# chrg127/stereomatching

Measured on AMD Instinct MI355X. Metric: Mpixel-disparities/s, higher is better.
Workload: dtype u32 bit-packed edges, i32 counts

## Files before the change

### stereomatching_amd/csrc/sm_bs_network.h

```cpp
#pragma once

#ifdef SM_BS_NETWORK_HOST
#include <cstdint>
typedef uint32_t u32;
#define SM_NET_FN inline
#define SM_NET_UNROLL
#define SM_PIN() do { } while (0)
#define SM_SYNC() do { } while (0)
template <int IMM>
inline u32 bop(u32 a, u32 b, u32 c)
{
    u32 r = 0;
    for (int k = 0; k < 8; k++)
        if ((IMM >> k) & 1) r |= ((k & 4) ? a : ~a) & ((k & 2) ? b : ~b) & ((k & 1) ? c : ~c);
    return r;
}
#else
#define SM_NET_FN __device__ __forceinline__
#define SM_NET_UNROLL _Pragma("unroll")
#endif

#include "sm_bs_ops.h"

struct NetCell { short a, b, c, s, cy; short imm; short w; bool grp = false; };

template <int N, int SB>
struct NetPlan {
    static constexpr int NIN = 2 * N + SB;
    static constexpr int MAXC = 2 * N + 2 * SB;
    NetCell cell[MAXC] = {};
    int ncell = 0;
    int nwires = NIN;
    int nops = 0;
    short out[SB] = {};
};

template <int N, int SB, bool GR = false>
constexpr NetPlan<N, SB> net_make_plan()
{
    NetPlan<N, SB> p;
    constexpr int G = GR ? N / 3 : 0;
    short q[4 * N + 4 * SB] = {}, nx[2 * N + 2 * SB] = {};
    bool qneg[4 * N + 4 * SB] = {}, nxneg[2 * N + 2 * SB] = {};
    short qgrp[4 * N + 4 * SB] = {};
    int head = 0, tail = 0, nn = 0;
    for (int w = 0; w < SB; w++) {
        const bool top = w == SB - 1;
        head = 0; tail = 0;
        q[tail] = (short)(2 * N + w); qneg[tail++] = false;
        if (w == 0) {
            for (int g = 0; g < G; g++) {
                qgrp[tail] = (short)(1 + 3 * g); qneg[tail++] = false;
                qgrp[tail] = (short)(1 + N + 3 * g); qneg[tail++] = true;
            }
            for (int i = 3 * G; i < N; i++) {
                q[tail] = (short)i; qneg[tail++] = false;
                q[tail] = (short)(N + i); qneg[tail++] = true;
            }
        }
        for (int i = 0; i < nn; i++) { q[tail] = nx[i]; qneg[tail++] = nxneg[i]; }
        nn = 0;
        while (tail - head >= 2) {
            const int k = tail - head >= 3 ? 3 : 2;
            for (int j = 0; j < k; j++)
                if (qgrp[head + j]) {
                    const short in0 = (short)(qgrp[head + j] - 1);
                    NetCell gc = {in0, (short)(in0 + 1), (short)(in0 + 2), -1, -1, BOP_MAJ_NC, (short)w, true};
                    gc.s = (short)p.nwires++;
                    gc.cy = (short)p.nwires++;
                    nx[nn] = gc.cy; nxneg[nn++] = qneg[head + j];
                    p.nops++;
                    q[head + j] = gc.s; qgrp[head + j] = 0;
                    p.cell[p.ncell++] = gc;
                }
            short in[3] = {-1, -1, -1};
            int np = 0, ng = 0;
            for (int j = 0; j < k; j++) if (!qneg[head + j]) in[np++] = q[head + j];
            for (int j = 0; j < k; j++) if (qneg[head + j]) in[np + ng++] = q[head + j];
            head += k;
            NetCell c = {in[0], in[1], in[2], (short)p.nwires++, -1, 0, (short)w};
            bool sneg = false, cneg = false;
            if (k == 3) {
                sneg = ng & 1; cneg = ng >= 2;
                c.imm = ng == 1 ? BOP_MAJ_NC : ng == 2 ? BOP_BORROW : BOP_MAJ;
            } else {
                sneg = ng == 2; cneg = ng >= 1;
                c.imm = ng == 1 ? BOP_ANDN : 0;
            }
            p.nops++;
            if (!top) {
                c.cy = (short)p.nwires++;
                nx[nn] = c.cy; nxneg[nn++] = cneg;
                p.nops++;
            }
            q[--head] = c.s; qneg[head] = sneg;
            p.cell[p.ncell++] = c;
        }
        p.out[w] = q[head];
        if (qneg[head] && !top) { nx[nn] = q[head]; nxneg[nn++] = true; }
    }
    bool made[NetPlan<N, SB>::NIN + 2 * NetPlan<N, SB>::MAXC] = {};
    for (int i = 0; i < NetPlan<N, SB>::NIN; i++) made[i] = true;
    NetCell order[NetPlan<N, SB>::MAXC] = {};
    bool done[NetPlan<N, SB>::MAXC] = {};
    for (int n = 0; n < p.ncell; n++) {
        int pick = -1;
        for (int i = 0; i < p.ncell; i++) {
            const NetCell &c = p.cell[i];
            if (done[i] || !made[c.a] || !made[c.b] || (c.c >= 0 && !made[c.c])) continue;
            if (pick < 0 || c.w > p.cell[pick].w) pick = i;
        }
        done[pick] = true;
        order[n] = p.cell[pick];
        made[order[n].s] = true;
        if (order[n].cy >= 0) made[order[n].cy] = true;
    }
    for (int n = 0; n < p.ncell; n++) p.cell[n] = order[n];
    return p;
}

template <int N, int SB, bool GR = false>
struct NetPlanOf { static constexpr NetPlan<N, SB> value = net_make_plan<N, SB, GR>(); };

template <int N, int SB, bool GR = false>
constexpr int net_min_distance(int it)
{
    const NetPlan<N, SB> p = NetPlanOf<N, SB, GR>::value;
    int pos[NetPlan<N, SB>::NIN + 2 * NetPlan<N, SB>::MAXC] = {};
    for (int i = 0; i < NetPlan<N, SB>::NIN; i++) pos[i] = -(1 << 20);
    int at = 0, best = 1 << 20;
    for (int n = 0; n < p.ncell; n++) {
        const NetCell &c = p.cell[n];
        const short in[3] = {c.a, c.b, c.c};
        for (int j = 0; j < 3; j++)
            if (in[j] >= 0 && at - pos[in[j]] < best) best = at - pos[in[j]];
        pos[c.s] = at;
        if (!c.grp) at += it;
        if (c.cy >= 0) { pos[c.cy] = at; at += it; }
    }
    return best;
}

template <int N, bool GR = false>
constexpr int net_ops() { return net_make_plan<N, bits_for(N * N), GR>().nops; }
constexpr int net_ops_count_tree(int n)
{
    int ops = 0, m = n;
    for (int w = 0; w < bits_for(n); w++) {
        int carries = 0;
        while (m >= 3) { ops += 2; m -= 2; carries++; }
        if (m == 2) { ops += 2; m = 1; carries++; }
        m = carries;
    }
    return ops;
}
constexpr int net_ops_addsub(int n)
{
    const int hb = bits_for(n), sb = bits_for(n * n);
    int ops = 2 + 2 * (hb - 1) + 2;
    for (int k = 1; k < sb; k++) ops += k + 1 < sb ? 2 : 1;
    return ops;
}
constexpr int net_ops_separate(int n) { return 2 * net_ops_count_tree(n) + net_ops_addsub(n); }

template <int N, int SB, int IT, int DS, int NW, int ID, typename XF>
SM_NET_FN u32 net_wire(const u32 (&S)[DS][SB], int dd0, XF &xin, const u32 (&wr)[IT][NW], int it)
{
    if constexpr (ID < 2 * N) return xin(it, ID);
    else if constexpr (ID < 2 * N + SB) return S[dd0 + it][ID - 2 * N];
    else return wr[it][ID - 2 * N - SB];
}

template <int N, int SB, int IT, int DS, bool GR, int C, int NW, typename XF>
SM_NET_FN void net_cells(u32 (&S)[DS][SB], int dd0, XF &xin, u32 (&wr)[IT][NW])
{
    constexpr NetPlan<N, SB> P = NetPlanOf<N, SB, GR>::value;
    if constexpr (C < P.ncell) {
        constexpr NetCell cl = P.cell[C];
        constexpr int NIN = 2 * N + SB;
        constexpr bool full = cl.c >= 0;
        u32 a[IT], b[IT], c[IT];
SM_NET_UNROLL
        for (int it = 0; it < IT; it++) {
            a[it] = net_wire<N, SB, IT, DS, NW, cl.a>(S, dd0, xin, wr, it);
            b[it] = net_wire<N, SB, IT, DS, NW, cl.b>(S, dd0, xin, wr, it);
            if constexpr (full) c[it] = net_wire<N, SB, IT, DS, NW, cl.c>(S, dd0, xin, wr, it);
            else c[it] = 0u;
        }
SM_NET_UNROLL
        for (int it = 0; it < IT; it++) {
            if constexpr (cl.grp) wr[it][cl.s - NIN] = c[it];
            else {
                if constexpr (full) wr[it][cl.s - NIN] = bop<BOP_XOR3>(a[it], b[it], c[it]);
                else wr[it][cl.s - NIN] = a[it] ^ b[it];
                SM_PIN();
            }
        }
        if constexpr (cl.cy >= 0) {
SM_NET_UNROLL
            for (int it = 0; it < IT; it++) {
                if constexpr (full || cl.imm != 0) wr[it][cl.cy - NIN] = bop<cl.imm>(a[it], b[it], c[it]);
                else wr[it][cl.cy - NIN] = a[it] & b[it];
                SM_PIN();
            }
        }
        SM_SYNC();
        net_cells<N, SB, IT, DS, GR, C + 1, NW>(S, dd0, xin, wr);
    }
}

template <int N, int SB, bool GR = false>
constexpr bool net_planes_from_cells()
{
    constexpr NetPlan<N, SB> P = NetPlanOf<N, SB, GR>::value;
    for (int k = 0; k < SB; k++)
        if (P.out[k] < 2 * N + SB) return false;
    return true;
}

template <int N, int SB, int IT, int DS, bool GR = false, typename XF>
SM_NET_FN void network_lockstep(u32 (&S)[DS][SB], int dd0, XF xin)
{
    constexpr NetPlan<N, SB> P = NetPlanOf<N, SB, GR>::value;
    constexpr int NIN = 2 * N + SB, NW = P.nwires - NIN;
    static_assert(net_planes_from_cells<N, SB, GR>(), "every plane of S' comes out of a cell");
    static_assert(net_min_distance<N, SB, GR>(IT) >= IT, "a cell reads a result made fewer than IT operations before");
    u32 wr[IT][NW];
    net_cells<N, SB, IT, DS, GR, 0, NW>(S, dd0, xin, wr);
SM_NET_UNROLL
    for (int k = 0; k < SB; k++)
SM_NET_UNROLL
        for (int it = 0; it < IT; it++) S[dd0 + it][k] = wr[it][P.out[k] - NIN];
}
```

### stereomatching_amd/csrc/sm_match_bs_kernel.h

```cpp

#pragma once
#include "sm_internal.h"

#ifndef SM_BS_TU
#error "define SM_BS_TU (a token naming the translation unit) before including this header"
#endif
#define SM_BS_CAT2(a, b) a##b
#define SM_BS_CAT(a, b) SM_BS_CAT2(a, b)

#define SM_BS_WAVES 2
#define SM_STAGE_CH_L 4
#define SM_STAGE_CH_R 5

#ifdef SM_STAMPS
static __device__ unsigned long long *g_sm_stamps;
int SM_BS_CAT(sm_bs_set_stamps_, SM_BS_TU)(void *buf)
{
    return hipMemcpyToSymbol(HIP_SYMBOL(g_sm_stamps), &buf, sizeof buf) == hipSuccess ? 0 : SM_ERR_HIP;
}
#define SM_STAMP(slot)                                                                          \
    do {                                                                                        \
        if ((threadIdx.x & 63) == 0 && g_sm_stamps) {                   \
            const size_t wg_ = (((size_t)blockIdx.z * gridDim.y + blockIdx.y) * gridDim.x + blockIdx.x) \
                               * (blockDim.x >> 6) + (threadIdx.x >> 6);                        \
            g_sm_stamps[wg_ * 10 + 2 * (slot)] = __builtin_amdgcn_s_memrealtime();              \
            g_sm_stamps[wg_ * 10 + 2 * (slot) + 1] = __builtin_amdgcn_s_memtime();              \
            if ((slot) == 0)                                                                    \
                g_sm_stamps[wg_ * 10 + 8] = ((unsigned long long)__builtin_amdgcn_s_getreg(63508) << 32) | \
                                            (unsigned)__builtin_amdgcn_s_getreg(63492);         \
        }                                                                                       \
    } while (0)
#else
#define SM_STAMP(slot) do { } while (0)
#endif

template <int IMM>
__device__ __forceinline__ u32 bop(u32 a, u32 b, u32 c)
{
    return __builtin_amdgcn_bitop3_b32(a, b, c, IMM);
}
#include "sm_bs_ops.h"

__device__ __forceinline__ u32 alignbit(u32 hi, u32 lo, u32 sh)
{
    return __builtin_amdgcn_alignbit(hi, lo, sh);
}

typedef unsigned long long u64;
struct RawRow { u64 l01; u32 l2; u64 r01, r23; };
struct RawCentre { u32 l; u64 r01; u32 r2; };
typedef __attribute__((address_space(3))) const volatile u32 lds_vu32;
typedef u64 __attribute__((aligned(4))) u64a4;
typedef __attribute__((address_space(3))) const volatile u64a4 lds_vu64;
__device__ __forceinline__ void lds_issue(RawRow &o, u32 aL, u32 aR)
{
    o.l01 = *(lds_vu64 *)(uintptr_t)aL;
    o.l2 = *(lds_vu32 *)(uintptr_t)(aL + 8);
    o.r01 = *(lds_vu64 *)(uintptr_t)aR;
    o.r23 = *(lds_vu64 *)(uintptr_t)(aR + 8);
}
__device__ __forceinline__ void lds_issue(RawCentre &o, u32 aL, u32 aR)
{
    o.l = *(lds_vu32 *)(uintptr_t)aL;
    o.r01 = *(lds_vu64 *)(uintptr_t)aR;
    o.r2 = *(lds_vu32 *)(uintptr_t)(aR + 8);
}

typedef int v4i __attribute__((ext_vector_type(4)));
__device__ __forceinline__ void store_map4(i32 *p, v4i v)
{
    asm volatile("global_store_dwordx4 %0, %1, off sc1\n\ts_nop 1" : : "v"(p), "v"(v) : "memory");
}

template <int SB, int HB>
__device__ __forceinline__ void add_planes(u32 (&s)[SB], const u32 (&h)[HB])
{
    u32 c = s[0] & h[0];
    s[0] ^= h[0];
#pragma unroll
    for (int k = 1; k < SB; k++) {
        if (k < HB) {
            const u32 cn = bop<BOP_MAJ>(s[k], h[k], c);
            s[k] = bop<BOP_XOR3>(s[k], h[k], c);
            c = cn;
        } else {
            const u32 cn = k + 1 < SB ? s[k] & c : 0u;
            s[k] ^= c;
            c = cn;
        }
    }
}

#define SM_PIN() __builtin_amdgcn_sched_barrier(0)
#define SM_SYNC() do { asm volatile("s_nop 0"); SM_PIN(); } while (0)

#include "sm_bs_network.h"

template <int N, int HB, int IT, typename XF>
__device__ __forceinline__ void count_lockstep(XF xin, u32 (&h)[IT][HB])
{
    u32 q[IT][2 * N + 2];
    int head = 0, tail = N;
#pragma unroll
    for (int w = 0; w < HB; w++) {
        u32 nx[IT][N + 1];
        int nn = 0;
#pragma unroll
        for (int adder = 0; adder < N; adder++) {
            if (tail - head >= 3) {
                u32 a[IT], b[IT], c[IT];
#pragma unroll
                for (int it = 0; it < IT; it++) {
                    const bool in0 = w == 0 && head < N, in1 = w == 0 && head + 1 < N, in2 = w == 0 && head + 2 < N;
                    a[it] = in0 ? xin(it, in0 ? head : 0) : q[it][head];
                    b[it] = in1 ? xin(it, in1 ? head + 1 : 0) : q[it][head + 1];
                    c[it] = in2 ? xin(it, in2 ? head + 2 : 0) : q[it][head + 2];
                }
#pragma unroll
                for (int it = 0; it < IT; it++) { q[it][tail] = bop<BOP_XOR3>(a[it], b[it], c[it]); SM_PIN(); }
#pragma unroll
                for (int it = 0; it < IT; it++) { nx[it][nn] = bop<BOP_MAJ>(a[it], b[it], c[it]); SM_PIN(); }
                SM_SYNC();
                head += 3; tail++; nn++;
            }
        }
        if (tail - head == 2) {
            u32 a[IT], b[IT];
#pragma unroll
            for (int it = 0; it < IT; it++) {
                const bool in0 = w == 0 && head < N, in1 = w == 0 && head + 1 < N;
                a[it] = in0 ? xin(it, in0 ? head : 0) : q[it][head];
                b[it] = in1 ? xin(it, in1 ? head + 1 : 0) : q[it][head + 1];
            }
#pragma unroll
            for (int it = 0; it < IT; it++) { q[it][tail] = a[it] ^ b[it]; SM_PIN(); }
#pragma unroll
            for (int it = 0; it < IT; it++) { nx[it][nn] = a[it] & b[it]; SM_PIN(); }
            head += 2; tail++; nn++;
        }
#pragma unroll
        for (int it = 0; it < IT; it++) {
            const bool in0 = w == 0 && head < N;
            h[it][w] = tail - head == 1 ? (in0 ? xin(it, in0 ? head : 0) : q[it][head]) : 0u;
        }
        head = 0; tail = 0;
#pragma unroll
        for (int i = 0; i < N + 1; i++)
            if (i < nn) {
#pragma unroll
                for (int it = 0; it < IT; it++) q[it][tail] = nx[it][i];
                tail++;
            }
    }
}

template <int SB, int HB, int GS, int DS>
__device__ __forceinline__ void add_lockstep(u32 (&S)[DS][SB], int dd0, const u32 (&h)[GS][HB])
{
    u32 c[GS];
#pragma unroll
    for (int g = 0; g < GS; g++) { c[g] = S[dd0 + g][0] & h[g][0]; SM_PIN(); }
#pragma unroll
    for (int g = 0; g < GS; g++) { S[dd0 + g][0] ^= h[g][0]; SM_PIN(); }
#pragma unroll
    for (int k = 1; k < SB; k++) {
        u32 cn[GS];
#pragma unroll
        for (int g = 0; g < GS; g++) {
            if (k + 1 < SB) { cn[g] = k < HB ? bop<BOP_MAJ>(S[dd0 + g][k], h[g][k], c[g]) : (S[dd0 + g][k] & c[g]); SM_PIN(); }
            else cn[g] = 0;
        }
#pragma unroll
        for (int g = 0; g < GS; g++) {
            if (k < HB) S[dd0 + g][k] = bop<BOP_XOR3>(S[dd0 + g][k], h[g][k], c[g]);
            else S[dd0 + g][k] ^= c[g];
            SM_PIN();
        }
#pragma unroll
        for (int g = 0; g < GS; g++) c[g] = cn[g];
        SM_SYNC();
    }
}

template <int V> struct IntTag { static constexpr int value = V; };

template <int T, int CH>
struct RowStager {
    const u32 *src;
    u32 *dst;
    int rw, total, step_k, step_from, wrap_from;
    int e, k, from;
    u32 v[CH];
    __device__ __forceinline__ RowStager(const u32 *src_, int stride, u32 *dst_, int nrow, int rw_)
        : src(src_), dst(dst_), rw(rw_), total(nrow * rw_)
    {
        const float inv = __builtin_amdgcn_rcpf((float)rw);
        const int t_row = (int)(((float)T + 0.5f) * inv), row = (int)(((float)threadIdx.x + 0.5f) * inv);
        step_k = T - t_row * rw;
        step_from = t_row * stride + step_k;
        wrap_from = stride - rw;
        e = (int)threadIdx.x;
        k = e - row * rw;
        from = row * stride + k;
    }
    __device__ __forceinline__ bool more() const { return e - (int)threadIdx.x + T * CH < total; }
    template <typename Tag>
    __device__ __forceinline__ void issue(Tag)
    {
#pragma unroll
        for (int j = 0; j < CH; j++) {
            v[j] = src[Tag::value && e >= total ? 0 : from];
            e += T; k += step_k; from += step_from;
            if (k >= rw) { k -= rw; from += wrap_from; }
        }
    }
    template <typename Tag>
    __device__ __forceinline__ void write(Tag) const
    {
#pragma unroll
        for (int j = 0; j < CH; j++) {
            const int ej = e - (CH - j) * T;
            dst[Tag::value && ej >= total ? 0 : ej] = v[j];
        }
    }
};

template <int CTRL>
__device__ __forceinline__ u32 dpp(u32 v)
{
    return (u32)__builtin_amdgcn_update_dpp(0, (int)v, CTRL, 0xf, 0xf, true);
}

template <int K>
__device__ __forceinline__ u32 from_partner(u32 v)
{
    if (K == 0) return dpp<0xB1>(v);
    if (K == 1) return dpp<0x4E>(v);
    if (K == 2) return dpp<0x141>(v);
    if (K == 3) return dpp<0x140>(v);
    return (u32)__shfl_xor((int)v, 1 << K);
}


template <int N, int DS, bool FULLD, bool GHOST, bool CAP2 = false, bool DUO = false>
__global__ __launch_bounds__(DUO ? 128 : 64, SM_BS_WAVES) void k_match_bs(const u32 *__restrict__ ext,
                                                 i32 *__restrict__ web, i32 *__restrict__ best,
                                                 const MatchGeom g)
{
    constexpr int HALF = N / 2;
    constexpr int HB = bits_for(N);
    constexpr int SB = bits_for(N * N);
    constexpr int AB = DS == 16 ? 4 : DS == 8 ? 3 : 2;
    constexpr int ABMAX = AB + 6;
    static_assert(SB <= 16, "window counts are moved through two byte lanes");
    static_assert((1 << SB) - 1 > N * N, "the all-ones marker must not be a real count");
    static_assert(N + DS - 1 + 31 < 96, "right window must fit three words");

    extern __shared__ __attribute__((aligned(16))) u32 lds[];
    if (CAP2) asm volatile("" ::: "v175");
    if (web == nullptr) return;
    const int tid = DUO ? (int)(threadIdx.x & 63u) : (int)threadIdx.x;
    const int wv = DUO ? __builtin_amdgcn_readfirstlane((int)(threadIdx.x >> 6)) : 0;
    const int pair = blockIdx.z;
    SM_STAMP(0);
    const unsigned slot_parity = __builtin_amdgcn_s_getreg(63492) & 1;
    unsigned long long clk = __builtin_amdgcn_s_memtime();
    constexpr unsigned PATTERN = DS == 16 ? 0xF0F0F0F0u : 0xAAAAAAAAu;
    const unsigned long long clk0 = clk;
#define SM_SLICE_PRIO()                                                               \
    do {                                                                              \
        const unsigned unit_ = (unsigned)((clk - clk0) >> 14) & 31u;                  \
        if (((PATTERN >> unit_) ^ slot_parity) & 1) __builtin_amdgcn_s_setprio(3);    \
        else __builtin_amdgcn_s_setprio(0);                                           \
    } while (0)
#define SM_SLICE_READ() do { clk = __builtin_amdgcn_s_memtime(); } while (0)
    int tile_x, tile_y;
    sm_xcd_tile(g.tiles_x, g.tiles_y, tile_x, tile_y);
    const int tx0 = tile_x * g.tw;
    const int ty0 = tile_y * (DUO ? 2 * g.tile_h : g.tile_h);
    const int plw = g.plw, prw = g.prw, nsr = g.nsr;
    const u32 *extL = ext + (size_t)pair * 2 * g.ext_image_words;
    u32 *pL = lds;
    u32 *pR = pL + nsr * plw;

    constexpr int T = DUO ? 128 : 64;
    const u32 *rowsL = extL + (size_t)ty0 * g.ext_words + (tx0 >> 5);
    RowStager<T, SM_STAGE_CH_L> stL(rowsL, g.ext_words, pL, nsr, plw);
    RowStager<T, SM_STAGE_CH_R> stR(rowsL + g.ext_image_words, g.ext_words, pR, nsr, prw);
    while (stL.more()) { stL.issue(IntTag<0>{}); stL.write(IntTag<0>{}); }
    stL.issue(IntTag<1>{});
    while (stR.more()) { stR.issue(IntTag<0>{}); stR.write(IntTag<0>{}); }
    stR.issue(IntTag<1>{});

    const int s = tid & (g.nl - 1);
    const int wi = tid >> g.log2nl;
    const int d0 = s * DS;
    const int x0 = tx0 + 32 * wi;
    const int bL = SM_PADT + 32 * wi - HALF, bR = bL + d0;
    const int wL = bL >> 5, shL = bL & 31, wR = bR >> 5, shR = bR & 31;
    const int bRc = SM_PADT + 32 * wi + d0;
    const int wRc = bRc >> 5, shRc = bRc & 31;
    const int wLc = 1 + wi;

    u32 cvv[N];
    if (GHOST) {
        const int lo = min(64, max(0, HALF - x0)), hi = min(64, max(0, g.w + HALF - x0));
        const unsigned long long below_hi = hi >= 64 ? ~0ull : (1ull << hi) - 1ull;
        const unsigned long long below_lo = lo >= 64 ? ~0ull : (1ull << lo) - 1ull;
        const unsigned long long cm = hi > lo ? below_hi & ~below_lo : 0ull;
        const u32 c0 = (u32)cm, c1 = (u32)(cm >> 32);
#pragma unroll
        for (int i = 0; i < N; i++) cvv[i] = i ? alignbit(c1, c0, i) : c0;
    }
    u32 dvalid = (1u << DS) - 1u;
    if (!FULLD) {
        const int dlim = g.D - d0;
        dvalid = dlim >= DS ? (1u << DS) - 1u : (dlim <= 0 ? 0u : ((1u << dlim) - 1u));
    }

    u32 S[DS][SB];
#pragma unroll
    for (int dd = 0; dd < DS; dd++)
#pragma unroll
        for (int k = 0; k < SB; k++) {
            S[dd][k] = 0;
            asm volatile("" : "+v"(S[dd][k]));
        }

    SM_PIN();
    stL.write(IntTag<1>{});
    stR.write(IntTag<1>{});
    __syncthreads();
    SM_STAMP(1);

    struct RowViews { u32 lv[N]; u32 rw[3]; };
    auto load_views = [&](int srow, RowViews &v) {
        const u32 *rl = pL + srow * plw + wL;
        const u32 *rr = pR + srow * prw + wR;
        const u32 l0 = alignbit(rl[1], rl[0], shL), l1 = alignbit(rl[2], rl[1], shL);
#pragma unroll
        for (int k = 0; k < 3; k++) v.rw[k] = alignbit(rr[k + 1], rr[k], shR);
#pragma unroll
        for (int i = 0; i < N; i++) v.lv[i] = i ? alignbit(l1, l0, i) : l0;
    };
    auto views_of = [&](const RawRow &q, RowViews &v) {
        const u32 a0 = (u32)q.l01, a1 = (u32)(q.l01 >> 32), a2 = q.l2;
        const u32 r0 = (u32)q.r01, r1 = (u32)(q.r01 >> 32), r2 = (u32)q.r23, r3 = (u32)(q.r23 >> 32);
        const u32 l0 = alignbit(a1, a0, shL), l1 = alignbit(a2, a1, shL);
        v.rw[0] = alignbit(r1, r0, shR); v.rw[1] = alignbit(r2, r1, shR); v.rw[2] = alignbit(r3, r2, shR);
#pragma unroll
        for (int i = 0; i < N; i++) v.lv[i] = i ? alignbit(l1, l0, i) : l0;
    };
    auto rview = [&](const RowViews &v, int j) -> u32 {
        return (j & 31) ? alignbit(v.rw[(j >> 5) + 1], v.rw[j >> 5], j & 31) : v.rw[j >> 5];
    };

    constexpr int GW = DS >= 4 ? 4 : DS;
    constexpr int GS = DS >= 4 ? 4 : DS;
    static_assert(DS % GW == 0 && DS % GS == 0, "shift groups");
    auto slide_in = [&](int srow) {
        RowViews v;
        load_views(srow, v);
        u32 rv[N + GW - 1];
#pragma unroll
        for (int m = 0; m < N - 1; m++) rv[m + GW] = rview(v, m);
#pragma unroll
        for (int dd0 = 0; dd0 < DS; dd0 += GW) {
#pragma unroll
            for (int m = 0; m < N - 1; m++) rv[m] = rv[m + GW];
#pragma unroll
            for (int m = 0; m < GW; m++) { rv[N - 1 + m] = rview(v, dd0 + N - 1 + m); SM_PIN(); }
            SM_SYNC();
            u32 h[GW][HB];
            count_lockstep<N, HB, GW>([&](int it, int i) -> u32 {
                const u32 x = GHOST ? bop<BOP_XOR_AND>(v.lv[i], rv[it + i], cvv[i]) : (v.lv[i] ^ rv[it + i]);
                SM_PIN();
                return x;
            }, h);
            add_lockstep<SB, HB, GW, DS>(S, dd0, h);
        }
    };
    constexpr int G = N / 3, RXK = 3 * (G - 1), RXW = RXK + GS;
    constexpr bool GROUPED = !GHOST && 2 * G * DS > 2 * G + 2 * (RXK + DS) && !(DS == 8 && N >= 19);
    auto slide_views = [&](const RowViews &vn, const RowViews &vo) {
        u32 rn[N + GS - 1], ro[N + GS - 1];
        u32 lxn[G], lxo[G], rxn[RXW], rxo[RXW];
#pragma unroll
        for (int m = 0; m < N - 1; m++) { rn[m + GS] = rview(vn, m); ro[m + GS] = rview(vo, m); }
        if (GROUPED) {
            SM_PIN(); SM_SYNC();
#pragma unroll
            for (int gq = 0; gq < G; gq++) {
                lxn[gq] = bop<BOP_XOR3>(vn.lv[3 * gq], vn.lv[3 * gq + 1], vn.lv[3 * gq + 2]); SM_PIN();
                lxo[gq] = bop<BOP_XOR3>(vo.lv[3 * gq], vo.lv[3 * gq + 1], vo.lv[3 * gq + 2]); SM_PIN();
            }
#pragma unroll
            for (int m = 0; m < RXK; m++) {
                rxn[m + GS] = bop<BOP_XOR3>(rn[m + GS], rn[m + GS + 1], rn[m + GS + 2]); SM_PIN();
                rxo[m + GS] = bop<BOP_XOR3>(ro[m + GS], ro[m + GS + 1], ro[m + GS + 2]); SM_PIN();
            }
        }
#pragma unroll
        for (int dd0 = 0; dd0 < DS; dd0 += GS) {
#pragma unroll
            for (int m = 0; m < N - 1; m++) { rn[m] = rn[m + GS]; ro[m] = ro[m + GS]; }
#pragma unroll
            for (int m = 0; m < GS; m++) {
                rn[N - 1 + m] = rview(vn, dd0 + N - 1 + m); SM_PIN();
                ro[N - 1 + m] = rview(vo, dd0 + N - 1 + m); SM_PIN();
            }
            SM_SYNC();
            if (GROUPED) {
#pragma unroll
                for (int m = 0; m < RXK; m++) { rxn[m] = rxn[m + GS]; rxo[m] = rxo[m + GS]; }
#pragma unroll
                for (int m = 0; m < GS; m++) { rxn[RXK + m] = bop<BOP_XOR3>(rn[RXK + m], rn[RXK + m + 1], rn[RXK + m + 2]); SM_PIN(); }
#pragma unroll
                for (int m = 0; m < GS; m++) { rxo[RXK + m] = bop<BOP_XOR3>(ro[RXK + m], ro[RXK + m + 1], ro[RXK + m + 2]); SM_PIN(); }
            }
            network_lockstep<N, SB, GS, DS, GROUPED>(S, dd0, [&](int it, int i) -> u32 {
                const int col = i < N ? i : i - N;
                if (GROUPED && col < 3 * G && col % 3 == 2) {
                    const u32 p = (i < N ? lxn[col / 3] : lxo[col / 3]) ^ (i < N ? rxn[it + col - 2] : rxo[it + col - 2]);
                    SM_PIN();
                    return p;
                }
                const u32 l = i < N ? vn.lv[col] : vo.lv[col];
                const u32 r = i < N ? rn[it + col] : ro[it + col];
                const u32 x = GHOST ? bop<BOP_XOR_AND>(l, r, cvv[col]) : (l ^ r);
                SM_PIN();
                return x;
            });
            SM_SYNC();
        }
    };

    const int mid = DUO ? min(ty0 + g.tile_h, g.h) : 0;
    const int sgn = DUO ? (wv ? 1 : -1) : 1;
    const int y0 = DUO ? (wv ? mid : mid - 1) : ty0;
    const int c0 = DUO ? y0 - ty0 + HALF : HALF;
    const int rows_out = DUO ? (wv ? min(ty0 + 2 * g.tile_h, g.h) - mid : mid - ty0)
                             : min(g.tile_h, g.h - ty0);

    SM_SLICE_PRIO();
    if (DUO) {
#pragma unroll 1
        for (int e = 0; e <= HALF; e++) {
        if (e == HALF) {
        constexpr int DH = DS / 2, XP = DH * SB / 2;
        static_assert(DS % 2 == 0 && (DH * SB) % 2 == 0, "exchange halves");
        typedef u32 v2u __attribute__((ext_vector_type(2)));
        v2u *xq = reinterpret_cast<v2u *>(lds + g.xm_off - XP * 128) + tid;
        auto exchange = [&](auto own_tag) {
            constexpr int OWN = decltype(own_tag)::value, OTH = 1 - OWN;
            v2u *slot_own = xq + OWN * XP * 64, *slot_oth = xq + OTH * XP * 64;
#pragma unroll
            for (int j = 0; j < XP; j++) {
                const int p = 2 * j, q = 2 * j + 1;
                const v2u v = {S[OTH * DH + p / SB][p % SB], S[OTH * DH + q / SB][q % SB]};
                slot_oth[j * 64] = v;
            }
            __syncthreads();
#pragma unroll
            for (int dd = 0; dd < DH; dd += 2) {
                u32 o[2][SB];
#pragma unroll
                for (int j = 0; j < SB; j++) {
                    const int p = 2 * j, q = 2 * j + 1;
                    const v2u v = slot_own[(dd * SB / 2 + j) * 64];
                    o[p / SB][p % SB] = v.x;
                    o[q / SB][q % SB] = v.y;
                }
                add_planes<SB, SB>(S[OWN * DH + dd], o[0]);
                add_planes<SB, SB>(S[OWN * DH + dd + 1], o[1]);
#pragma unroll
                for (int j = 0; j < SB; j++) {
                    const int p = 2 * j, q = 2 * j + 1;
                    const v2u v = {S[OWN * DH + dd + p / SB][p % SB], S[OWN * DH + dd + q / SB][q % SB]};
                    slot_own[(dd * SB / 2 + j) * 64] = v;
                }
            }
            __syncthreads();
#pragma unroll
            for (int j = 0; j < XP; j++) {
                const int p = 2 * j, q = 2 * j + 1;
                const v2u v = slot_oth[j * 64];
                S[OTH * DH + p / SB][p % SB] = v.x;
                S[OTH * DH + q / SB][q % SB] = v.y;
            }
        };
        if (wv) exchange(IntTag<1>{}); else exchange(IntTag<0>{});
        }
        slide_in(c0 + sgn * e);
        }
        if (rows_out <= 0) return;
    } else {
#pragma unroll 1
        for (int e = 0; e < N; e++) slide_in(e);
    }
    SM_SLICE_READ();
    SM_STAMP(2);

    u32 *xm_base = lds + g.xm_off - ((DUO && wv) ? g.xm_words : 0);
    u32 *xm_wbase = xm_base + (s & 3) * ((SB + AB + 3) / 4) * 256;
    const u32 xm_wunit = (u32)(wi * (g.nl >> 2) + (s >> 2) + 2 * (s & 3));
    const u32 ldsL = (u32)(uintptr_t)pL, ldsR = (u32)(uintptr_t)pR;
    const u32 sL = (u32)(sgn * 4 * plw), sR = (u32)(sgn * 4 * prw);
    u32 aNewL = ldsL + 4u * wL + sL * (HALF + 1) + 4u * plw * c0, aNewR = ldsR + 4u * wR + sR * (HALF + 1) + 4u * prw * c0;
    u32 aCenL = ldsL + 4u * wLc + 4u * plw * c0, aCenR = ldsR + 4u * wRc + 4u * prw * c0;
    RawRow qn, qo;
    RawCentre qc;
    lds_issue(qc, aCenL, aCenR);
    if (!DUO || rows_out > 1) {
        lds_issue(qn, aNewL, aNewR);
        lds_issue(qo, aNewL - sL * N, aNewR - sR * N);
    }
#pragma unroll 1
    for (int t = 0;;) {
        SM_SLICE_PRIO();
        const int y = y0 + sgn * t;
        const u32 lc = qc.l;
        const u32 c0_ = (u32)qc.r01, c1_ = (u32)(qc.r01 >> 32), c2_ = qc.r2;
        const u32 rc0 = alignbit(c1_, c0_, shRc), rc1 = alignbit(c2_, c1_, shRc);

        u32 B[SB], arg[ABMAX];
#pragma unroll
        for (int k = 0; k < ABMAX; k++) arg[k] = 0;
        {
            constexpr int Q = 4, QS = DS / Q;
            constexpr int AQ = AB - 2;
            u32 Bq[Q][SB], aq[Q][AQ > 0 ? AQ : 1];
#pragma unroll
            for (int i = 0; i < QS; i++) {
                u32 upd[Q];
                u32 rcd[Q];
#pragma unroll
                for (int qd = 0; qd < Q; qd++) {
                    const int dd = qd * QS + i;
                    rcd[qd] = dd ? alignbit(rc1, rc0, dd) : rc0; SM_PIN();
                }
                SM_SYNC();
                if (i == 0) {
#pragma unroll
                    for (int qd = 0; qd < Q; qd++) {
                        upd[qd] = bop<BOP_XNOR>(lc, rcd[qd], 0u); SM_PIN();
                        if (!FULLD) { upd[qd] &= (u32)__builtin_amdgcn_sbfe((int)dvalid, qd * QS + i, 1); SM_PIN(); }
                    }
#pragma unroll
                    for (int k = 0; k < SB; k++)
#pragma unroll
                        for (int qd = 0; qd < Q; qd++) { Bq[qd][k] = bop<BOP_ORN>(upd[qd], S[qd * QS + i][k], 0u); SM_PIN(); }
#pragma unroll
                    for (int a = 0; a < AQ; a++)
#pragma unroll
                        for (int qd = 0; qd < Q; qd++) aq[qd][a] = 0;
                } else {
                    u32 bw[Q];
#pragma unroll
                    for (int k = 0; k < SB; k++)
#pragma unroll
                        for (int qd = 0; qd < Q; qd++) {
                            bw[qd] = bop<BOP_BORROW>(Bq[qd][k], S[qd * QS + i][k], k ? bw[qd] : 0u); SM_PIN();
                            if (qd == Q - 1 && (k & 1)) SM_SYNC();
                        }
#pragma unroll
                    for (int qd = 0; qd < Q; qd++) {
                        upd[qd] = bop<BOP_UPD>(lc, rcd[qd], bw[qd]); SM_PIN();
                        if (!FULLD) { upd[qd] &= (u32)__builtin_amdgcn_sbfe((int)dvalid, qd * QS + i, 1); SM_PIN(); }
                    }
#pragma unroll
                    for (int k = 0; k < SB; k++)
#pragma unroll
                        for (int qd = 0; qd < Q; qd++) {
                            Bq[qd][k] = bop<BOP_SEL>(upd[qd], S[qd * QS + i][k], Bq[qd][k]); SM_PIN();
                            if (qd == Q - 1 && (k & 1)) SM_SYNC();
                        }
#pragma unroll
                    for (int a = 0; a < AQ; a++)
#pragma unroll
                        for (int qd = 0; qd < Q; qd++) {
                            if ((i >> a) & 1) aq[qd][a] |= upd[qd]; else aq[qd][a] = bop<BOP_ANDN>(upd[qd], aq[qd][a], 0u);
                            SM_PIN();
                        }
                }
            }
            u32 bwm[2] = {0, 0};
#pragma unroll
            for (int k = 0; k < SB; k++)
#pragma unroll
                for (int m = 0; m < 2; m++) {
                    bwm[m] = bop<BOP_BORROW>(Bq[2 * m][k], Bq[2 * m + 1][k], k ? bwm[m] : 0u); SM_PIN();
                }
            u32 Bh[2][SB], ah[2][AQ + 1];
            u32 bwf = 0;
#pragma unroll
            for (int k = 0; k < SB; k++) {
#pragma unroll
                for (int m = 0; m < 2; m++) { Bh[m][k] = bop<BOP_SEL>(bwm[m], Bq[2 * m][k], Bq[2 * m + 1][k]); SM_PIN(); }
                if (k < AQ) {
#pragma unroll
                    for (int m = 0; m < 2; m++) { ah[m][k] = bop<BOP_SEL>(bwm[m], aq[2 * m][k], aq[2 * m + 1][k]); SM_PIN(); }
                }
                if (k > 0) { bwf = bop<BOP_BORROW>(Bh[0][k - 1], Bh[1][k - 1], k > 1 ? bwf : 0u); SM_PIN(); }
            }
#pragma unroll
            for (int k = SB; k < AQ; k++)
#pragma unroll
                for (int m = 0; m < 2; m++) { ah[m][k] = bop<BOP_SEL>(bwm[m], aq[2 * m][k], aq[2 * m + 1][k]); SM_PIN(); }
            ah[0][AQ] = ~bwm[0]; SM_PIN();
            ah[1][AQ] = ~bwm[1]; SM_PIN();
            bwf = bop<BOP_BORROW>(Bh[0][SB - 1], Bh[1][SB - 1], SB > 1 ? bwf : 0u); SM_PIN();
#pragma unroll
            for (int k = 0; k < SB; k++) { B[k] = bop<BOP_SEL>(bwf, Bh[0][k], Bh[1][k]); SM_PIN(); }
#pragma unroll
            for (int k = 0; k <= AQ; k++) { arg[k] = bop<BOP_SEL>(bwf, ah[0][k], ah[1][k]); SM_PIN(); }
            arg[AQ + 1] = ~bwf; SM_PIN();
        }

        auto emit_pixels = [&](u32 (&B)[SB], u32 (&arg)[ABMAX], int xw, int yy, int pfirst, int per, int pstep) {
            const int cw = per < 4 ? per : 4;
            const u32 cmask = (1u << cw) - 1u;
            u32 allone = B[0];
#pragma unroll
            for (int k = 1; k < SB; k++) allone &= B[k];
            u32 dm1 = (u32)(g.D - 1);
            asm volatile("" : "+s"(dm1));
#pragma unroll
            for (int k = 0; k < ABMAX; k++) {
                if (k >= AB && k >= AB + g.log2nl) continue;
                arg[k] = bop<BOP_SEL>(allone, (u32)-(i32)((dm1 >> k) & 1u), arg[k]);
            }
            for (int c = 0, p0 = pfirst; c < per; c += 4, p0 += pstep) {
                u32 bb = 0, bhi = 0, alo = 0, ahi = 0;
                if (best) {
#pragma unroll
                    for (int k = 0; k < SB; k++) {
                        const u32 sp = __umul24((B[k] >> p0) & cmask, 0x204081u) & 0x01010101u;
                        if (k < 8) bb += sp << k; else bhi += sp << (k - 8);
                    }
                }
#pragma unroll
                for (int k = 0; k < ABMAX; k++) {
                    if (k >= AB && k >= AB + g.log2nl) continue;
                    const u32 sp = __umul24((arg[k] >> p0) & cmask, 0x204081u) & 0x01010101u;
                    if (k < 8) alo += sp << k; else ahi += sp << (k - 8);
                }
                const u32 none = __umul24((allone >> p0) & cmask, 0x204081u) & 0x01010101u;
                i32 wv[4], bv[4];
#pragma unroll
                for (int q = 0; q < 4; q++) {
                    const bool no = (none >> (8 * q)) & 1u;
                    int taps = N * N;
                    if (GHOST) {
                        const int x = xw + p0 + q;
                        const int cols = min(g.w - 1, x + HALF) - max(0, x - HALF) + 1;
                        const int rws = min(g.h - 1, yy + HALF) - max(0, yy - HALF) + 1;
                        taps = cols * rws;
                    }
                    const i32 a = (i32)(((alo >> (8 * q)) & 255u) | (((ahi >> (8 * q)) & 255u) << 8));
                    wv[q] = a + 1;
                    bv[q] = no ? 0 : taps - (i32)(((bb >> (8 * q)) & 255u) | (((bhi >> (8 * q)) & 255u) << 8));
                }
                const int x = xw + p0;
                const size_t o = ((size_t)pair * g.h + yy) * g.w + x;
                const bool vec = cw == 4 && g.vec_ok && x + 4 <= g.w;
                if (g.web_bytes == 4) {
                    if (vec) {
                        const v4i wq = {wv[0], wv[1], wv[2], wv[3]};
                        store_map4(web + o, wq);
                    } else {
#pragma unroll
                        for (int q = 0; q < 4; q++)
                            if (q < cw && x + q < g.w) web[o + q] = wv[q];
                    }
                } else if (g.web_bytes == 1) {
                    u8 *web8 = reinterpret_cast<u8 *>(web);
                    if (vec) {
                        u32 pk = 0;
#pragma unroll
                        for (int q = 0; q < 4; q++) pk |= (u32)(wv[q] & 255) << (8 * q);
                        __builtin_nontemporal_store(pk, reinterpret_cast<u32 *>(web8 + o));
                    } else {
#pragma unroll
                        for (int q = 0; q < 4; q++)
                            if (q < cw && x + q < g.w) web8[o + q] = (u8)wv[q];
                    }
                } else {
                    unsigned short *web16 = reinterpret_cast<unsigned short *>(web);
                    if (vec) {
                        typedef u32 v2u __attribute__((ext_vector_type(2)));
                        const v2u pk = {(u32)wv[0] | ((u32)wv[1] << 16), (u32)wv[2] | ((u32)wv[3] << 16)};
                        __builtin_nontemporal_store(pk, reinterpret_cast<v2u *>(web16 + o));
                    } else {
#pragma unroll
                        for (int q = 0; q < 4; q++)
                            if (q < cw && x + q < g.w) web16[o + q] = (unsigned short)wv[q];
                    }
                }
                if (best) {
                    if (vec) {
                        const v4i bq = {bv[0], bv[1], bv[2], bv[3]};
                        store_map4(best + o, bq);
                    } else {
#pragma unroll
                        for (int q = 0; q < 4; q++)
                            if (q < cw && x + q < g.w) best[o + q] = bv[q];
                    }
                }
            }
        };

#define SM_MERGE(K, me, NA)                                                            \
        {                                                                              \
            u32 pb[SB], pa[NA];                                                        \
            _Pragma("unroll") for (int k = 0; k < SB; k++) pb[k] = from_partner<K>(B[k]);      \
            _Pragma("unroll") for (int k = 0; k < NA; k++) pa[k] = from_partner<K>(arg[k]);    \
            SM_PIN(); SM_SYNC();                                                       \
            const u32 mine_high = ((me) >> K) & 1 ? 0xffffffffu : 0u;                  \
            u32 bw = mine_high;           \
            bw = ~bw;                       \
            _Pragma("unroll") for (int k = 0; k < SB; k++) bw = bop<BOP_BORROW>(pb[k], B[k], bw); \
            const u32 take = bw;                                                       \
            _Pragma("unroll") for (int k = 0; k < SB; k++) B[k] = bop<BOP_SEL>(take, pb[k], B[k]); \
            _Pragma("unroll") for (int k = 0; k < NA; k++) arg[k] = bop<BOP_SEL>(take, pa[k], arg[k]); \
            arg[NA] = take ^ mine_high;                 \
        }
        if (g.xmerge) {
            constexpr int NPL = SB + AB, NPG = (NPL + 3) / 4;
            typedef u32 v4u __attribute__((ext_vector_type(4)));
            typedef __attribute__((address_space(3))) const volatile v4u lds_vv4;
            const u32 xm_lds = (u32)(uintptr_t)xm_base;
            const int r = t & 3;
            {
                u32 pl[4 * NPG];
#pragma unroll
                for (int k = 0; k < 4 * NPG; k++) pl[k] = k < SB ? B[k] : (k < NPL ? arg[k - SB] : 0u);
                const u32 unit = (xm_wunit + 16u * (u32)r) & 63u;
#pragma unroll
                for (int pg = 0; pg < NPG; pg++) {
                    const v4u v = {pl[4 * pg], pl[4 * pg + 1], pl[4 * pg + 2], pl[4 * pg + 3]};
                    *reinterpret_cast<v4u *>(xm_wbase + pg * 256 + unit * 4) = v;
                }
            }
            if (r == 3 || t + 1 >= rows_out) {
                __builtin_amdgcn_fence(__ATOMIC_RELEASE, "wavefront");
                __builtin_amdgcn_wave_barrier();
                const int lpi = g.nl >> 2, l2lpi = g.log2nl - 2;
                const int rr = tid >> 4, wr = (tid & 15) >> l2lpi, sub = tid & (lpi - 1);
                u32 Bm[SB], am[ABMAX];
#pragma unroll
                for (int k = 0; k < ABMAX; k++) am[k] = 0;
                v4u ev[4][NPG];
#pragma unroll
                for (int j = 0; j < 4; j++) {
                    const u32 unit = ((u32)tid + 2u * j) & 63u;
#pragma unroll
                    for (int pg = 0; pg < NPG; pg++)
                        ev[j][pg] = *(lds_vv4 *)(uintptr_t)(xm_lds + 4u * (u32)((j * NPG + pg) * 256) + 16u * unit);
                }
                SM_PIN();
#pragma unroll
                for (int j = 0; j < 4; j++) {
                    u32 e[4 * NPG];
#pragma unroll
                    for (int pg = 0; pg < NPG; pg++) {
                        const v4u v = ev[j][pg];
                        e[4 * pg] = v.x; e[4 * pg + 1] = v.y; e[4 * pg + 2] = v.z; e[4 * pg + 3] = v.w;
                    }
                    if (j == 0) {
#pragma unroll
                        for (int k = 0; k < SB; k++) Bm[k] = e[k];
#pragma unroll
                        for (int k = 0; k < AB; k++) am[k] = e[SB + k];
                    } else {
                        u32 bw = 0xffffffffu;
#pragma unroll
                        for (int k = 0; k < SB; k++) bw = bop<BOP_BORROW>(e[k], Bm[k], bw);
                        const u32 take = bw;
#pragma unroll
                        for (int k = 0; k < SB; k++) Bm[k] = bop<BOP_SEL>(take, e[k], Bm[k]);
#pragma unroll
                        for (int k = 0; k < AB; k++) am[k] = bop<BOP_SEL>(take, e[SB + k], am[k]);
                        if (j & 1) am[AB] |= take; else am[AB] = bop<BOP_ANDN>(take, am[AB], 0u);
                        if (j & 2) am[AB + 1] |= take; else am[AB + 1] = bop<BOP_ANDN>(take, am[AB + 1], 0u);
                    }
                }
                {
                    u32 (&B)[SB] = Bm;
                    u32 (&arg)[ABMAX] = am;
                    if (lpi > 1) SM_MERGE(0, sub, AB + 2)
                    if (lpi > 2) SM_MERGE(1, sub, AB + 3)
                    if (lpi > 4) SM_MERGE(2, sub, AB + 4)
                }
                const int tt = t - r + rr;
                const int yy = y0 + sgn * tt;
                if (rr <= r && yy < g.h && yy >= 0) {
                    const int per = 32 >> l2lpi;
                    emit_pixels(Bm, am, tx0 + 32 * wr, yy, 4 * sub, per, 4 * lpi);
                }
                __builtin_amdgcn_wave_barrier();
            }
        } else {
            if (g.nl > 1) SM_MERGE(0, s, AB)
            if (g.nl > 2) SM_MERGE(1, s, AB + 1)
            if (g.nl > 4) SM_MERGE(2, s, AB + 2)
            if (g.nl > 8) SM_MERGE(3, s, AB + 3)
            if (g.nl > 16) SM_MERGE(4, s, AB + 4)
            if (g.nl > 32) SM_MERGE(5, s, AB + 5)
            if (y < g.h) {
                const int per = 32 >> g.log2nl;
                emit_pixels(B, arg, x0, y, s * per, per, 4);
            }
        }
#undef SM_MERGE

        SM_SYNC();
        if (++t >= rows_out) break;
        {
            RowViews vn, vo;
            views_of(qn, vn);
            views_of(qo, vo);
            aNewL += sL; aNewR += sR; aCenL += sL; aCenR += sR;
            lds_issue(qc, aCenL, aCenR);
            if (t + 1 < rows_out) {
                lds_issue(qn, aNewL, aNewR);
                lds_issue(qo, aNewL - sL * N, aNewR - sR * N);
            }
            SM_SLICE_READ();
            SM_PIN(); SM_SYNC();
            slide_views(vn, vo);
        }
    }
    SM_STAMP(3);
}


template <int N, int DS, bool CAP2, bool DUO = false>
static const void *bs_ptr4(bool fulld, bool ghost)
{
    return fulld ? (ghost ? (const void *)k_match_bs<N, DS, true, true, CAP2, DUO> : (const void *)k_match_bs<N, DS, true, false, CAP2, DUO>)
                 : (ghost ? (const void *)k_match_bs<N, DS, false, true, CAP2, DUO> : (const void *)k_match_bs<N, DS, false, false, CAP2, DUO>);
}
template <int N, int DS, bool CAPPABLE>
static const void *bs_ptr(bool fulld, bool ghost, bool cap2)
{
    if (cap2) return CAPPABLE ? bs_ptr4<N, DS, CAPPABLE>(fulld, ghost) : nullptr;
    return bs_ptr4<N, DS, false>(fulld, ghost);
}
```

### stereomatching_amd/valu_model.py

```python
from __future__ import annotations

import json
from pathlib import Path

COUNTS = Path(__file__).resolve().parent / "valu_counts.json"


def variant_key(geom: dict, num_shifts: int, border: int, want_best: bool) -> str:
    fulld = geom["shift_lanes"] * geom["shifts_per_lane"] == num_shifts
    duo = ":duo" if geom["kernel"] == 4 and geom.get("waves_per_workgroup", 1) == 2 else ""
    cap2 = ":cap2" if geom["kernel"] == 4 and geom.get("two_wave_variant") else ""
    xm = ":xm" if geom["kernel"] == 4 and geom.get("lane_merge_lds") else ""
    return (f"k{geom['kernel']}:n{geom['window']}:ds{geom['shifts_per_lane']}:nl{geom['shift_lanes']}:"
            f"{'ghost' if border else 'toroidal'}:fulld{int(fulld)}:best{int(bool(want_best))}{duo}{cap2}{xm}")


def waves_and_rows(geom: dict, height: int, pairs: int):
    waves_per_wg = geom.get("waves_per_workgroup") or max(1, geom["threads"] // 64)
    waves = geom["tiles_x"] * geom["tiles_y"] * pairs * waves_per_wg
    rows = geom["tiles_x"] * height * pairs * (1 if geom["kernel"] == 4 else waves_per_wg)
    return waves, rows


def _setup_text(geom: dict) -> str:
    n = geom["window"]
    if geom["kernel"] == 4 and geom.get("waves_per_workgroup", 1) == 2:
        return (f"set-up + {n // 2 + 1} warm-up rows + swap of the {n - 1} shared rows' sums with the "
                f"workgroup's other wave")
    return f"set-up + {n} warm-up rows"


def match_launch(geom: dict, width: int, height: int, num_shifts: int, border: int,
                 pairs: int, want_best: bool = False):
    if not COUNTS.exists():
        return None
    table = json.loads(COUNTS.read_text())
    key = variant_key(geom, num_shifts, border, want_best)
    c = table.get("variants", {}).get(key)
    if not c:
        return None
    waves, rows = waves_and_rows(geom, height, pairs)
    total = c["per_wave"] * waves + c["per_wave_row"] * rows
    return {
        "wave_instructions": int(round(total)),
        "model": f"{waves} waves x {c['per_wave']:.0f} ({_setup_text(geom)}) + "
                 f"{rows} wave-rows x {c['per_wave_row']:.0f}",
        "source": f"{table.get('source', 'valu_counts.json')}; fit residual <= "
                  f"{c.get('max_rel_residual', 0) * 100:.2f} % over tile heights "
                  f"{[p[0] for p in c.get('fit_points', [])]}",
        "variant": key,
    }
```

Before: 12.43 million.

## Count shared warm-up rows with one carry-save counter tree in duo kernel

```diff
diff --git a/stereomatching_amd/csrc/sm_bs_network.h b/stereomatching_amd/csrc/sm_bs_network.h
--- a/stereomatching_amd/csrc/sm_bs_network.h
+++ b/stereomatching_amd/csrc/sm_bs_network.h
@@ -232,3 +232,157 @@
 SM_NET_UNROLL
         for (int it = 0; it < IT; it++) S[dd0 + it][k] = wr[it][P.out[k] - NIN];
 }
+
+struct CountCell { short a, b, c, s, cy, w; };
+
+template <int NI, int TB>
+struct CountPlan {
+    static constexpr int MAXC = NI + TB;
+    CountCell cell[MAXC] = {};
+    int ncell = 0;
+    int nwires = NI;
+    int nops = 0;
+    short out[TB] = {};
+};
+
+template <int NI, int TB>
+constexpr CountPlan<NI, TB> count_make_plan()
+{
+    static_assert(NI >= 3 && (1 << TB) > NI, "planes of the count");
+    CountPlan<NI, TB> p;
+    short q[2 * NI + 2 * TB] = {}, nx[NI + TB] = {};
+    int head = 0, tail = 0, nn = 0;
+    for (int w = 0; w < TB; w++) {
+        const bool top = w == TB - 1;
+        head = 0; tail = 0;
+        if (w == 0)
+            for (int i = 0; i < NI; i++) q[tail++] = (short)i;
+        for (int i = 0; i < nn; i++) q[tail++] = nx[i];
+        nn = 0;
+        while (tail - head >= 2) {
+            const int k = tail - head >= 3 ? 3 : 2;
+            CountCell c = {q[head], q[head + 1], (short)(k == 3 ? q[head + 2] : -1), (short)p.nwires++, -1, (short)w};
+            head += k;
+            p.nops++;
+            if (!top) {
+                c.cy = (short)p.nwires++;
+                nx[nn++] = c.cy;
+                p.nops++;
+            }
+            q[--head] = c.s;
+            p.cell[p.ncell++] = c;
+        }
+        p.out[w] = tail > head ? q[head] : (short)-1;
+    }
+    bool made[NI + 2 * CountPlan<NI, TB>::MAXC] = {};
+    for (int i = 0; i < NI; i++) made[i] = true;
+    CountCell order[CountPlan<NI, TB>::MAXC] = {};
+    bool done[CountPlan<NI, TB>::MAXC] = {};
+    for (int n = 0; n < p.ncell; n++) {
+        int pick = -1;
+        for (int i = 0; i < p.ncell; i++) {
+            const CountCell &c = p.cell[i];
+            if (done[i] || !made[c.a] || !made[c.b] || (c.c >= 0 && !made[c.c])) continue;
+            if (pick < 0 || c.w > p.cell[pick].w) pick = i;
+        }
+        done[pick] = true;
+        order[n] = p.cell[pick];
+        made[order[n].s] = true;
+        if (order[n].cy >= 0) made[order[n].cy] = true;
+    }
+    for (int n = 0; n < p.ncell; n++) p.cell[n] = order[n];
+    return p;
+}
+
+template <int NI, int TB>
+struct CountPlanOf { static constexpr CountPlan<NI, TB> value = count_make_plan<NI, TB>(); };
+
+template <int NI, int TB>
+constexpr int count_min_distance(int it)
+{
+    const CountPlan<NI, TB> p = CountPlanOf<NI, TB>::value;
+    int pos[NI + 2 * CountPlan<NI, TB>::MAXC] = {};
+    for (int i = 0; i < NI; i++) pos[i] = -(1 << 20);
+    int at = 0, best = 1 << 20;
+    for (int n = 0; n < p.ncell; n++) {
+        const CountCell &c = p.cell[n];
+        const short in[3] = {c.a, c.b, c.c};
+        for (int j = 0; j < 3; j++)
+            if (in[j] >= 0 && at - pos[in[j]] < best) best = at - pos[in[j]];
+        pos[c.s] = at;
+        at += it;
+        if (c.cy >= 0) { pos[c.cy] = at; at += it; }
+    }
+    return best;
+}
+
+constexpr int warm_ops_tree(int n, int cells_ops) { return n / 2 * n + cells_ops; }
+template <int N>
+constexpr int warm_ops_tree() { return warm_ops_tree(N, count_make_plan<N / 2 * N, bits_for(N / 2 * N)>().nops); }
+constexpr int warm_ops_rows(int n) { return n / 2 * (n + net_ops_count_tree(n) + 2 * bits_for(n * n) - 1); }
+
+template <int NI, int IT, int NW, int ID, typename XF>
+SM_NET_FN u32 count_wire(XF &xin, const u32 (&wr)[IT][NW], int it)
+{
+    if constexpr (ID < NI) return xin(it, ID);
+    else return wr[it][ID - NI];
+}
+
+template <int NI, int TB, int IT, int C, int NW, typename XF>
+SM_NET_FN void count_cells(XF &xin, u32 (&wr)[IT][NW])
+{
+    constexpr CountPlan<NI, TB> P = CountPlanOf<NI, TB>::value;
+    if constexpr (C < P.ncell) {
+        constexpr CountCell cl = P.cell[C];
+        constexpr bool full = cl.c >= 0;
+        u32 a[IT], b[IT], c[IT];
+SM_NET_UNROLL
+        for (int it = 0; it < IT; it++) {
+            a[it] = count_wire<NI, IT, NW, cl.a>(xin, wr, it);
+            b[it] = count_wire<NI, IT, NW, cl.b>(xin, wr, it);
+            if constexpr (full) c[it] = count_wire<NI, IT, NW, cl.c>(xin, wr, it);
+            else c[it] = 0u;
+        }
+SM_NET_UNROLL
+        for (int it = 0; it < IT; it++) {
+            if constexpr (full) wr[it][cl.s - NI] = bop<BOP_XOR3>(a[it], b[it], c[it]);
+            else wr[it][cl.s - NI] = a[it] ^ b[it];
+            SM_PIN();
+        }
+        if constexpr (cl.cy >= 0) {
+SM_NET_UNROLL
+            for (int it = 0; it < IT; it++) {
+                if constexpr (full) wr[it][cl.cy - NI] = bop<BOP_MAJ>(a[it], b[it], c[it]);
+                else wr[it][cl.cy - NI] = a[it] & b[it];
+                SM_PIN();
+            }
+        }
+        SM_SYNC();
+        count_cells<NI, TB, IT, C + 1, NW>(xin, wr);
+    }
+}
+
+template <int NI, int TB, int IT, int K, int NW>
+SM_NET_FN void count_planes(u32 (&h)[IT][TB], const u32 (&wr)[IT][NW])
+{
+    if constexpr (K < TB) {
+        constexpr CountPlan<NI, TB> P = CountPlanOf<NI, TB>::value;
+SM_NET_UNROLL
+        for (int it = 0; it < IT; it++) {
+            if constexpr (P.out[K] >= NI) h[it][K] = wr[it][P.out[K] - NI];
+            else h[it][K] = 0u;
+        }
+        count_planes<NI, TB, IT, K + 1, NW>(h, wr);
+    }
+}
+
+template <int NI, int TB, int IT, typename XF>
+SM_NET_FN void count_chain_lockstep(XF xin, u32 (&h)[IT][TB])
+{
+    constexpr CountPlan<NI, TB> P = CountPlanOf<NI, TB>::value;
+    constexpr int NW = P.nwires - NI;
+    static_assert(count_min_distance<NI, TB>(IT) >= IT, "a cell reads a result made fewer than IT operations before");
+    u32 wr[IT][NW];
+    count_cells<NI, TB, IT, 0, NW>(xin, wr);
+    count_planes<NI, TB, IT, 0, NW>(h, wr);
+}
diff --git a/stereomatching_amd/csrc/sm_match_bs_kernel.h b/stereomatching_amd/csrc/sm_match_bs_kernel.h
--- a/stereomatching_amd/csrc/sm_match_bs_kernel.h
+++ b/stereomatching_amd/csrc/sm_match_bs_kernel.h
@@ -183,6 +183,11 @@
 }
 
 template <int V> struct IntTag { static constexpr int value = V; };
+
+constexpr bool warm_tree_taken(int n, bool duo)
+{
+    return duo && n / 2 >= 2 && n <= 13;
+}
 
 template <int T, int CH>
 struct RowStager {
@@ -318,14 +323,18 @@
         dvalid = dlim >= DS ? (1u << DS) - 1u : (dlim <= 0 ? 0u : ((1u << dlim) - 1u));
     }
 
+    constexpr int TB = bits_for(HALF * N);
+    constexpr bool WT = warm_tree_taken(N, DUO);
     u32 S[DS][SB];
-#pragma unroll
-    for (int dd = 0; dd < DS; dd++)
-#pragma unroll
-        for (int k = 0; k < SB; k++) {
-            S[dd][k] = 0;
-            asm volatile("" : "+v"(S[dd][k]));
-        }
+    if constexpr (!WT) {
+#pragma unroll
+        for (int dd = 0; dd < DS; dd++)
+#pragma unroll
+            for (int k = 0; k < SB; k++) {
+                S[dd][k] = 0;
+                asm volatile("" : "+v"(S[dd][k]));
+            }
+    }
 
     SM_PIN();
     stL.write(IntTag<1>{});
@@ -444,35 +453,76 @@
 
     SM_SLICE_PRIO();
     if (DUO) {
+        if constexpr (WT) {
+            static_assert(TB <= SB, "the count of HALF rows fits the sum planes");
+            static_assert(warm_ops_tree<N>() < warm_ops_rows(N), "the counter is the shorter form");
+            static_assert(N != 9 || (warm_ops_tree<N>() == 104 && warm_ops_rows(N) == 144), "operations per shift at 9 x 9");
+            const u32 a0L = (u32)(uintptr_t)pL + 4u * (u32)(c0 * plw + wL), a0R = (u32)(uintptr_t)pR + 4u * (u32)(c0 * prw + wR);
+            const u32 stL_ = (u32)(sgn * 4 * plw), stR_ = (u32)(sgn * 4 * prw);
+            RawRow raw[HALF];
+#pragma unroll
+            for (int r = 0; r < HALF; r++) lds_issue(raw[r], a0L + stL_ * (u32)r, a0R + stR_ * (u32)r);
+            SM_PIN();
+            RowViews v[HALF];
+            u32 rv[HALF][N + GW - 1];
+#pragma unroll
+            for (int r = 0; r < HALF; r++) {
+                views_of(raw[r], v[r]);
+#pragma unroll
+                for (int m = 0; m < N - 1; m++) rv[r][m + GW] = rview(v[r], m);
+            }
+#pragma unroll
+            for (int dd0 = 0; dd0 < DS; dd0 += GW) {
+#pragma unroll
+                for (int r = 0; r < HALF; r++) {
+#pragma unroll
+                    for (int m = 0; m < N - 1; m++) rv[r][m] = rv[r][m + GW];
+#pragma unroll
+                    for (int m = 0; m < GW; m++) { rv[r][N - 1 + m] = rview(v[r], dd0 + N - 1 + m); SM_PIN(); }
+                }
+                SM_SYNC();
+                u32 h[GW][TB];
+                count_chain_lockstep<HALF * N, TB, GW>([&](int it, int i) -> u32 {
+                    const int r = i / N, col = i % N;
+                    const u32 x = GHOST ? bop<BOP_XOR_AND>(v[r].lv[col], rv[r][it + col], cvv[col]) : (v[r].lv[col] ^ rv[r][it + col]);
+                    SM_PIN();
+                    return x;
+                }, h);
+#pragma unroll
+                for (int it = 0; it < GW; it++)
+#pragma unroll
+                    for (int k = 0; k < SB; k++) S[dd0 + it][k] = k < TB ? h[it][k] : 0u;
+            }
+        }
 #pragma unroll 1
-        for (int e = 0; e <= HALF; e++) {
+        for (int e = WT ? HALF : 0; e <= HALF; e++) {
         if (e == HALF) {
-        constexpr int DH = DS / 2, XP = DH * SB / 2;
-        static_assert(DS % 2 == 0 && (DH * SB) % 2 == 0, "exchange halves");
+        constexpr int DH = DS / 2, XP = DH * SB / 2, PB = WT ? TB : SB, XQ = DH * PB / 2;
+        static_assert(DS % 2 == 0 && (DH * SB) % 2 == 0 && (DH * PB) % 2 == 0, "exchange halves");
         typedef u32 v2u __attribute__((ext_vector_type(2)));
         v2u *xq = reinterpret_cast<v2u *>(lds + g.xm_off - XP * 128) + tid;
         auto exchange = [&](auto own_tag) {
             constexpr int OWN = decltype(own_tag)::value, OTH = 1 - OWN;
             v2u *slot_own = xq + OWN * XP * 64, *slot_oth = xq + OTH * XP * 64;
 #pragma unroll
-            for (int j = 0; j < XP; j++) {
+            for (int j = 0; j < XQ; j++) {
                 const int p = 2 * j, q = 2 * j + 1;
-                const v2u v = {S[OTH * DH + p / SB][p % SB], S[OTH * DH + q / SB][q % SB]};
-                slot_oth[j * 64] = v;
+                const v2u v = {S[OTH * DH + p / PB][p % PB], S[OTH * DH + q / PB][q % PB]};
+                slot_oth[(XP - XQ + j) * 64] = v;
             }
             __syncthreads();
 #pragma unroll
             for (int dd = 0; dd < DH; dd += 2) {
-                u32 o[2][SB];
-#pragma unroll
-                for (int j = 0; j < SB; j++) {
+                u32 o[2][PB];
+#pragma unroll
+                for (int j = 0; j < PB; j++) {
                     const int p = 2 * j, q = 2 * j + 1;
-                    const v2u v = slot_own[(dd * SB / 2 + j) * 64];
-                    o[p / SB][p % SB] = v.x;
-                    o[q / SB][q % SB] = v.y;
-                }
-                add_planes<SB, SB>(S[OWN * DH + dd], o[0]);
-                add_planes<SB, SB>(S[OWN * DH + dd + 1], o[1]);
+                    const v2u v = slot_own[(XP - XQ + dd * PB / 2 + j) * 64];
+                    o[p / PB][p % PB] = v.x;
+                    o[q / PB][q % PB] = v.y;
+                }
+                add_planes<SB, PB>(S[OWN * DH + dd], o[0]);
+                add_planes<SB, PB>(S[OWN * DH + dd + 1], o[1]);
 #pragma unroll
                 for (int j = 0; j < SB; j++) {
                     const int p = 2 * j, q = 2 * j + 1;
diff --git a/stereomatching_amd/valu_model.py b/stereomatching_amd/valu_model.py
--- a/stereomatching_amd/valu_model.py
+++ b/stereomatching_amd/valu_model.py
@@ -25,6 +25,9 @@
 def _setup_text(geom: dict) -> str:
     n = geom["window"]
     if geom["kernel"] == 4 and geom.get("waves_per_workgroup", 1) == 2:
+        if 5 <= n <= 13:
+            return (f"set-up + one counter over {n // 2} shared warm-up rows + 1 warm-up row + swap of the {n - 1} "
+                    f"shared rows' sums with the workgroup's other wave")
         return (f"set-up + {n // 2 + 1} warm-up rows + swap of the {n - 1} shared rows' sums with the "
                 f"workgroup's other wave")
     return f"set-up + {n} warm-up rows"
```

New measurement: 12.58 million, median of 6. +1.2%, better.
